# gmarcais/Jellyfish

Hardware: NVIDIA H100
Metric: k-mers counted/sec at k=21 (higher is better)
Workload: dtype u64

## Files before the change

### jellyfish_b200/csrc/jf_engine.cu

```cuda
#include <cuda_runtime.h>
#include <algorithm>
#include <atomic>
#include <cmath>
#include <cstdio>
#include <cstring>
#include <string>
#include <type_traits>
#include <utility>
#include <vector>

#include "../../include/jfgpu.h"
#include "host/jf_matrix.hpp"
#include "jf_kernels.cuh"
#include "jf_extract.cuh"
#include "jf_window.cuh"
#include "jf_dump.cuh"
#include "jf_shard.cuh"
#include "jf_query.cuh"
#include "jf_wide.cuh"
#include "jf_bloom.cuh"
#include "jf_sam.cuh"
#include "jf_newline.cuh"

using namespace jfk;
// ... 399 lines not shown
template<int NTH>
size_t count_smem_bytes(size_t lut_bytes, size_t stage_bytes, size_t bloom_bytes = 0, bool fast = false) {
  const size_t part = fast ? FAST_SMEM : (stage_bytes ? PMAX * 4 + stage_bytes : 0);
  return ((sizeof(ExtractSmemT<NTH>) + 15) & ~(size_t)15) + lut_bytes + part + bloom_bytes;
}

int ensure_scratch(jfgpu_engine* e, uint64_t n_tiles) {
  if(n_tiles <= e->scratch_tiles) return JFGPU_OK;
  uint64_t want = std::max<uint64_t>(n_tiles, 1024);
  CUDA_OK(e, cudaStreamSynchronize(e->cs));
  e->scratch_tiles = 0;
  CUDA_OK(e, make_all(need(e->nlA, want * 8), need(e->nlB, want * 8), need(e->cntA, want * 4), need(e->cntB, want * 4), need(e->tstate, want)));
  e->scratch_tiles = want;
  return JFGPU_OK;
}

uint32_t ring_len_for(uint32_t P) {
  uint32_t p2 = 1; while(p2 < P) p2 <<= 1;
  const uint32_t len = p2 >= RING_P ? RING : RING * (RING_P / p2);
  return std::min<uint32_t>(len, 1024);
}
PartDev part_dev(const jfgpu_engine* e) {
  PartDev d;
  memset(&d, 0, sizeof(d));
  const PartState& ps = e->part;
  d.P = ps.P; d.region_bits = ps.region_bits; d.rec_bytes = ps.rec_bytes; d.cap = ps.cap; d.flush_min = ps.flush_min;
  d.chunk_recs = CHUNK_BYTES / std::max(1u, ps.rec_bytes); d.n_chunks = ps.n_chunks; d.stage_bytes = ps.stage_bytes;
  d.margin = ps.margin;
  d.lazy_win = e->tab.materialized < e->tab.local_size ? e->tab.win_state.as<uint32_t>() : nullptr;
  d.arena_chunks = ps.arena_chunks;
  d.ring_len = ring_len_for(ps.P ? ps.P : 1);
  d.pool = ps.pool.as<uint8_t>(); d.pool_next = ps.pool_next.as<unsigned int>(); d.n_units = d.pool_next + ps.n_arenas; d.dir = ps.dir.as<uint2>();
  d.cta_chunk = ps.cta_chunk.as<uint32_t>(); d.cta_fill = ps.cta_fill.as<uint32_t>();
  d.spill_keys = ps.spill_keys.as<uint64_t>(); d.spill_counts = ps.spill_counts.as<uint64_t>();
  d.spill_n = ps.spill_n.as<unsigned long long>(); d.spill_cap = ps.spill_cap;
  return d;
}

PartDev shard_send_dev(const jfgpu_engine* e, int bank) {
  PartDev d;
  memset(&d, 0, sizeof(d));
  const ShardState& sh = e->sh;
  const uint32_t G = e->p.n_shards;
  d.P = sh.P; d.region_bits = sh.sbits; d.rec_bytes = 4; d.chunk_recs = CHUNK_BYTES / 4;
  d.n_chunks = (uint32_t)(sh.arena_chunks * G); d.arena_chunks = (uint32_t)sh.arena_chunks;
  d.by_owner = 1; d.owner_shift = sh.owner_shift;
  d.ring_len = ring_len_for(sh.P);
  { const double mean = 4096.0 / sh.P; d.margin = std::max<uint32_t>(2 * RING, (uint32_t)(mean + 6.0 * sqrt(mean) + 8.0)); }
  d.pool = sh.send_pool + (size_t)bank * G * sh.arena_chunks * CHUNK_BYTES;
  d.dir = sh.send_dir + (size_t)bank * G * sh.arena_chunks;
  d.pool_next = sh.pool_next[bank].as<unsigned int>(); d.n_units = d.pool_next + G;
  d.cta_chunk = sh.cta_chunk.as<uint32_t>(); d.cta_fill = sh.cta_fill.as<uint32_t>();
  return d;
}

void part_configure(jfgpu_engine* e) {
  PartState& ps = e->part;
  const Table& t = e->tab;
  ps.P = 0;
  if(e->kw == 4) return;
  if(e->p.no_partition || t.bytes() < ((size_t)(e->p.part_min_mb ? e->p.part_min_mb : 256) << 20)) return;
  uint32_t P = 256;
  const size_t region_target = (size_t)(e->p.region_mb ? e->p.region_mb : 64) << 20;
  const size_t owned_bytes = (size_t)t.local_size * (t.slot_bits / 8);
  while(P < (uint32_t)PMAX && (owned_bytes / P) > region_target) P <<= 1;
  if(t.slot_bits == 32 && t.local_lsize > ceil_log2(P)) {
    const uint32_t bits = t.local_lsize - ceil_log2(P) + t.hb, extra = bits > 32 ? bits - 32 : 0;
    if(extra && extra < 8 && (P << extra) <= (uint32_t)RING_P && t.local_lsize - ceil_log2(P << extra) > WIN_LG) P <<= extra;
  }
  for(;; P >>= 1) {
    if(P < 64 || t.local_lsize < 8 || (1u << (t.local_lsize - 8)) < P) return;
    const uint32_t region_bits = t.local_lsize - ceil_log2(P);
    const uint32_t bits = region_bits + t.hb;
    const uint32_t rec = bits <= 32 ? 4 : bits <= 64 ? 8 : bits <= 128 ? 16 : 0;
    if(!rec) return;
    const double mean = 1024.0 * 32 / P;
    const uint32_t margin = (uint32_t)(mean + 6.0 * sqrt(mean) + 8.0);
    if(margin * 2 > CHUNK_BYTES / rec) return;
    ps.P = P; ps.region_bits = region_bits; ps.rec_bytes = rec; ps.cap = 0; ps.flush_min = 0; ps.margin = margin;
    ps.stage_bytes = PMAX * 4;
    return;
  }
}

int part_alloc(jfgpu_engine* e) {
  PartState& ps = e->part;
  if(ps.pool.p) return JFGPU_OK;
  size_t free_b = 0, total_b = 0;
  CUDA_OK(e, cudaMemGetInfo(&free_b, &total_b));
  size_t want = e->p.pool_bytes ? (size_t)e->p.pool_bytes : std::min<size_t>((size_t)(free_b * 0.7), (size_t)64 << 30);
  const size_t floor_b = (size_t)e->n_sm * ps.P * CHUNK_BYTES * 2;
  if(want < floor_b) want = floor_b;
  ps.n_arenas = (uint32_t)e->n_sm;
  ps.arena_chunks = (uint32_t)std::min<size_t>(want / CHUNK_BYTES / ps.n_arenas, 0xFFFFFFF0u / ps.n_arenas);
  ps.n_chunks = ps.arena_chunks * ps.n_arenas;
  ps.spill_cap = (uint64_t)16 << 20;
  if(make_all(need(ps.pool, (size_t)ps.n_chunks * CHUNK_BYTES), need(ps.dir, (size_t)ps.n_chunks * 8), need(ps.order, (size_t)ps.n_chunks * 4),
              need(ps.pool_next, ((size_t)ps.n_arenas + 2) * 4), need(ps.cta_chunk, (size_t)e->n_sm * PMAX * 4),
              need(ps.cta_fill, (size_t)e->n_sm * PMAX * 4), need(ps.spill_keys, ps.spill_cap * 8 * e->kw), need(ps.spill_counts, ps.spill_cap * 8),
              need(ps.spill_n, 8), need(ps.hist, PMAX * 12), need(ps.start, PMAX * 4), need(ps.cursor, PMAX * 4), need(ps.unit_cursor, 8)) != cudaSuccess)
    return fail(e, JFGPU_ERR_NOMEM, "device allocation of the record pool failed");
  CUDA_OK(e, cudaMemsetAsync(ps.pool_next.p, 0, ps.pool_next.bytes, e->cs));
  CUDA_OK(e, cudaMemsetAsync(ps.spill_n.p, 0, 8, e->cs));
  CUDA_OK(e, cudaMemsetAsync(ps.cta_chunk.p, 0xFF, ps.cta_chunk.bytes, e->cs));
  CUDA_OK(e, cudaMemsetAsync(ps.cta_fill.p, 0, ps.cta_fill.bytes, e->cs));
  ps.bound_chunks = ps.P;
  ps.pending = false;
  CUDA_OK(e, cudaStreamSynchronize(e->cs));
  return JFGPU_OK;
}

static unsigned long long* region_recs(PartState& ps) { return reinterpret_cast<unsigned long long*>(ps.hist.as<uint32_t>() + PMAX); }

int regrow(jfgpu_engine* e);
int spill_table(jfgpu_engine* e, uint64_t n_failed);
int read_stats(jfgpu_engine* e);
int bloom_draw(jfgpu_engine* e);
BloomDev bloom_dev(const jfgpu_engine* e);

struct FailWatch {
  jfgpu_engine* e; cudaStream_t st;
  unsigned n = 0;
  bool step(bool last) {
    const int slot = (int)(n++ & 1);
    cudaMemcpyAsync(e->h_watch + slot, e->stats.as<unsigned long long>() + STAT_FAILED, 8, cudaMemcpyDeviceToHost, st);
    cudaEventRecord(e->ev_watch[slot], st);
    return (n > 1 && seen(slot ^ 1)) || (last && seen(slot));
  }
  bool seen(int slot) { cudaEventSynchronize(e->ev_watch[slot]); return e->h_watch[slot] != 0; }
};
static cudaError_t win_event(jfgpu_engine* e, cudaStream_t st) {
  if(e->wev_used == e->wev.size()) e->wev.emplace_back();
  Event& ev = e->wev[e->wev_used];
  if(!ev) { const cudaError_t c = make_all(need(ev, cudaEventDefault)); if(c != cudaSuccess) return c; }
  cudaEventRecord(ev, st);
  e->wev_used++;
  return cudaSuccess;
}
static void resolve_win_events(jfgpu_engine* e, cudaStream_t st) {
  const size_t n_groups = e->wev_used / 4;
  std::vector<uint32_t> flag(n_groups);
  if(n_groups && (cudaMemcpyAsync(flag.data(), e->part.w_flag.p, n_groups * 4, cudaMemcpyDeviceToHost, st) != cudaSuccess ||
                  cudaStreamSynchronize(st) != cudaSuccess)) cudaGetLastError();
  for(size_t j = 0; j < n_groups; ++j)
    for(int q = 0; q < 3; ++q) {
      float ms = 0;
      const int to = q == 0 ? 1 : q == 1 ? (flag[j] ? 0 : 1) : 2;
      if(cudaEventElapsedTime(&ms, e->wev[4 * j + q], e->wev[4 * j + q + 1]) == cudaSuccess) e->win_ms[to] += ms; else cudaGetLastError();
    }
  e->wev_used = 0;
}
static bool window_enabled(jfgpu_engine* e, const PartDev& pd) {
  return (e->p.k2_mode == 0 || e->p.k2_mode == 3 || e->p.k2_mode == 4) && e->op == 0 && e->tab.slot_bits == 32 && pd.rec_bytes == 4 &&
         pd.region_bits > WIN_LG && pd.region_bits - WIN_LG <= 11 && CHUNK_BYTES == (WIN_ST_NTH / 2) * 16;
}
static bool lazy_zero_ok(jfgpu_engine* e) {
  return e->part.P && e->bloom.mode == BLOOM_NONE && window_enabled(e, part_dev(e)) &&
         tri(e->tab.max_reprobe) < ((uint64_t)1 << e->part.region_bits);
}
int part_drain(jfgpu_engine* e, cudaStream_t st) {
  PartState& ps = e->part;
  if(!ps.P || !ps.pool.p || !ps.pending) return JFGPU_OK;
  PartDev pd = part_dev(e);
  const bool win = window_enabled(e, pd);
  const int g = e->n_sm * 4;
  if(!e->ev_d0) CUDA_OK(e, make_all(need(e->ev_d0, cudaEventDefault), need(e->ev_d1, cudaEventDefault)));
  cudaEventRecord(e->ev_d0, st);
  close_chunks_kernel<<<g, 256, 0, st>>>(pd, (uint32_t)e->n_sm); JF_LAUNCHED();
  CUDA_OK(e, cudaMemsetAsync(ps.hist.p, 0, PMAX * 12, st));
  chunk_hist_kernel<<<g, 256, 0, st>>>(pd, ps.hist.as<uint32_t>(), win ? region_recs(ps) : nullptr); JF_LAUNCHED();
  chunk_scan_kernel<<<1, 1024, 0, st>>>(pd.P, ps.hist.as<uint32_t>(), ps.start.as<uint32_t>(), ps.cursor.as<uint32_t>(), pd.n_units); JF_LAUNCHED();
  chunk_scatter_kernel<<<g, 256, 0, st>>>(pd, ps.cursor.as<uint32_t>(), ps.order.as<uint32_t>()); JF_LAUNCHED();
  CUDA_OK(e, cudaMemsetAsync(ps.unit_cursor.p, 0, 8, st));
  const TableDev T0 = table_dev(e, e->tab);
  const bool careful = e->p.allow_regrow != 0 || e->spill_fn != nullptr;
  unsigned int n_units = 0xFFFFFFFFu;
  if(careful || win) {
    CUDA_OK(e, cudaMemcpyAsync(&n_units, pd.n_units, 4, cudaMemcpyDeviceToHost, st));
    CUDA_OK(e, cudaStreamSynchronize(st));
    n_units = std::min(n_units, ps.n_chunks);
  }
  const unsigned group = careful ? (unsigned)std::max<uint64_t>(1, e->fail_group / pd.chunk_recs) : 0xFFFFFFFFu;

  const uint32_t wpr_lg = win ? pd.region_bits - WIN_LG : 0;
  const uint64_t wpr = (uint64_t)1 << wpr_lg;
  const size_t scatter_smem = ((size_t)4 * wpr + (size_t)WIN_ST_UNITS * pd.chunk_recs) * 4;
  std::vector<uint32_t> start(pd.P + 1);
  std::vector<unsigned long long> recs(pd.P);
  auto win_begin = [&]() -> int {
    if(!ps.w_rec.p) {
      ps.w_rec_cap = (uint64_t)64 << 20;
      ps.w_def_cap = WIN_DEF_CAP;
      if(make_all(need(ps.w_rec, ps.w_rec_cap * 4 + 64), need(ps.w_start, (((size_t)WIN_MAX_G << 11) + 1) * 4), need(ps.w_cursor, ((size_t)WIN_MAX_G << 11) * 4),
                  need(ps.w_cnt, ((size_t)WIN_MAX_G << 11) * 4), need(ps.w_def_n, 16), need(ps.w_flag, PMAX * 4),
                  need(ps.w_def_pos[0], ps.w_def_cap * 8), need(ps.w_def_high[0], ps.w_def_cap * 4),
                  need(ps.w_def_pos[1], ps.w_def_cap * 8), need(ps.w_def_high[1], ps.w_def_cap * 4)) != cudaSuccess)
        return fail(e, JFGPU_ERR_NOMEM, "device allocation of the window buffers failed");
      CUDA_OK(e, cudaMemsetAsync(ps.w_def_n.p, 0, 16, st));
    }
    CUDA_OK(e, cudaMemsetAsync(ps.w_flag.p, e->p.k2_mode == 3 ? 1 : 0, PMAX * 4, st));
    CUDA_OK(e, cudaMemcpyAsync(start.data(), ps.start.p, (size_t)pd.P * 4, cudaMemcpyDeviceToHost, st));
    CUDA_OK(e, cudaMemcpyAsync(recs.data(), region_recs(ps), (size_t)pd.P * 8, cudaMemcpyDeviceToHost, st));
    CUDA_OK(e, cudaStreamSynchronize(st));
    start[pd.P] = n_units;
    for(uint32_t r = 0; r < pd.P; ++r) start[r] = std::min(start[r], n_units);
    cudaFuncSetAttribute(win_scatter_kernel<true>, cudaFuncAttributeMaxDynamicSharedMemorySize, (int)scatter_smem);
    cudaFuncSetAttribute(win_scatter_kernel<false>, cudaFuncAttributeMaxDynamicSharedMemorySize, (int)scatter_smem);
    return JFGPU_OK;
  };
  int rc = win ? win_begin() : JFGPU_OK;
  auto bucket_cap = [&](uint64_t m) -> uint64_t {
    const uint64_t c = e->p.k2_mode == 4 ? m : m + (uint64_t)std::ceil(6.0 * std::sqrt((double)m)) + 16;
    return (c + 3) & ~(uint64_t)3;
  };
  bool zero = win && e->tab.materialized == 0;
  int def_wait = -1;
  auto run_deferred = [&](int set) {
    WinDev wd;
    memset(&wd, 0, sizeof(wd));
    wd.def_pos = ps.w_def_pos[set].as<uint64_t>(); wd.def_high = ps.w_def_high[set].as<uint32_t>();
    wd.def_n = ps.w_def_n.as<unsigned long long>() + set; wd.def_cap = ps.w_def_cap;
    if(e->kw == 1) win_deferred_kernel<1><<<e->n_sm * 2, 256, 0, st>>>(T0, wd, e->tab.inv_lut.as<uint64_t>(), e->nbytes);
    else           win_deferred_kernel<2><<<e->n_sm * 2, 256, 0, st>>>(T0, wd, e->tab.inv_lut.as<uint64_t>(), e->nbytes);
    JF_LAUNCHED();
    cudaMemsetAsync(wd.def_n, 0, 8, st);
  };
  auto end_zero = [&]() -> int {
    const int rc2 = table_materialize(e, e->tab, st);
    if(rc2 || !zero) return rc2;
    if(def_wait >= 0) run_deferred(def_wait);
    def_wait = -1; zero = false;
    return JFGPU_OK;
  };
  DevBuf old_inv;
  bool rebuilt = false;
  auto range = [&](unsigned done, unsigned upto) -> int {
    int rc2 = end_zero();
    if(rc2) return rc2;
    cudaMemsetAsync(ps.unit_cursor.p, 0, 8, st);
    const TableDev T = table_dev(e, e->tab);
    if(rebuilt) {
      const size_t smem = (size_t)e->nbytes * 256 * 8 * 2;
      rc2 = dispatch(e, e->kw, e->tab.slot_bits, [&](auto KW, auto SB) -> int {
        auto kern = rehash_chunks_kernel<decltype(KW)::value, decltype(SB)::value>;
        cudaFuncSetAttribute(kern, cudaFuncAttributeMaxDynamicSharedMemorySize, (int)smem);
        kern<<<e->n_sm, 512, smem, st>>>(T, T0, pd, ps.order.as<uint32_t>(), ps.unit_cursor.as<unsigned int>(), done, upto,
                                        old_inv.as<uint64_t>(), e->tab.lut.as<uint64_t>(), e->nbytes);
        return JFGPU_OK;
      });
    } else if(e->op == 0 && e->tab.slot_bits == 32 && pd.rec_bytes == 4 && e->p.k2_mode != 2) {
      if(e->kw == 1) insert_chunks32_kernel<1><<<e->n_sm * 2, 768, 0, st>>>(T, pd, ps.order.as<uint32_t>(), ps.unit_cursor.as<unsigned int>(), done, upto, e->tab.inv_lut.as<uint64_t>(), e->nbytes);
      else           insert_chunks32_kernel<2><<<e->n_sm * 2, 768, 0, st>>>(T, pd, ps.order.as<uint32_t>(), ps.unit_cursor.as<unsigned int>(), done, upto, e->tab.inv_lut.as<uint64_t>(), e->nbytes);
    } else
      rc2 = dispatch(e, e->kw, e->tab.slot_bits, [&](auto KW, auto SB) -> int {
        insert_chunks_kernel<decltype(KW)::value, decltype(SB)::value><<<e->n_sm * 2, 512, 0, st>>>(
            T, pd, ps.order.as<uint32_t>(), ps.unit_cursor.as<unsigned int>(), done, upto, e->tab.inv_lut.as<uint64_t>(), e->nbytes);
        return JFGPU_OK;
      });
    if(!rc2) JF_LAUNCHED();
    return rc2;
  };

  FailWatch watch{e, st};
  unsigned done = 0;
  uint32_t r0 = 0, ng = 0;
  bool ranged = false;
  while(!rc) {
    const bool window = win && !rebuilt;
    if(done >= n_units && (window || ranged)) break;
    unsigned upto = 0;
    if(!window) {
      upto = (unsigned)std::min<uint64_t>((uint64_t)done + group, n_units);
      rc = range(done, upto);
      ranged = true;
    } else {
      WinDev wd;
      memset(&wd, 0, sizeof(wd));
      uint32_t G = 0, stiles = 0;
      uint64_t m = 0, cap = 0;
      while(r0 + G < pd.P && G < WIN_MAX_G) {
        const uint32_t nu = start[r0 + G + 1] - start[r0 + G];
        if(careful && start[r0 + G + 1] - start[r0] > group) break;
        const uint64_t m2 = std::max<uint64_t>(m, (recs[r0 + G] + wpr - 1) / wpr), cap2 = bucket_cap(m2);
        if((G + 1) * wpr * std::max(cap2, m2 + 3) > ps.w_rec_cap) break;
        m = m2; cap = cap2;
        wd.stile_first[G] = stiles; wd.unit_first[G] = start[r0 + G];
        stiles += (nu + WIN_ST_UNITS - 1) / WIN_ST_UNITS;
        ++G;
      }
      if(G == 0) {
        upto = start[r0 + 1]; r0 += 1;
        rc = range(done, upto);
      } else {
        wd.stile_first[G] = stiles; wd.unit_first[G] = start[r0 + G];
        wd.g0 = r0; wd.G = G; wd.wpr_lg = wpr_lg; wd.n_tiles = stiles; wd.cap = (uint32_t)cap;
        wd.overflow = ps.w_flag.as<uint32_t>() + e->wev_used / 4;
        wd.wstart = ps.w_start.as<uint32_t>(); wd.wcursor = ps.w_cursor.as<uint32_t>(); wd.wcnt = ps.w_cnt.as<uint32_t>();
        wd.wrec = ps.w_rec.as<uint32_t>(); wd.wrec_cap = ps.w_rec_cap;
        const int set = zero ? (int)(ng & 1) : 0;
        wd.def_pos = ps.w_def_pos[set].as<uint64_t>(); wd.def_high = ps.w_def_high[set].as<uint32_t>();
        wd.def_n = ps.w_def_n.as<unsigned long long>() + set; wd.def_cap = ps.w_def_cap;
        wd.lazy_win = zero ? e->tab.win_state.as<uint32_t>() : nullptr;
        const uint32_t hb = e->tab.fbits - e->tab.rbits;
        auto settle = [&]() {
          if(!zero) { if(stiles) run_deferred(set); return; }
          e->tab.materialized = (uint64_t)(r0 + G) << pd.region_bits;
          if(def_wait >= 0) run_deferred(def_wait);
          def_wait = stiles ? set : -1;
        };
        ++ng;
        if(stiles) {
          CUDA_OK(e, cudaMemsetAsync(ps.w_cursor.p, 0, ((size_t)G << wpr_lg) * 4, st));
          CUDA_OK(e, win_event(e, st));
          win_scatter_kernel<true><<<stiles, WIN_ST_NTH, scatter_smem, st>>>(pd, wd, ps.order.as<uint32_t>(), hb); JF_LAUNCHED();
          win_scan_kernel<<<1, 1024, 0, st>>>(wd, T0.stats); JF_LAUNCHED();
          CUDA_OK(e, win_event(e, st));
          win_scatter_kernel<false><<<std::min<uint32_t>(stiles, e->n_sm * 2), WIN_ST_NTH, scatter_smem, st>>>(pd, wd, ps.order.as<uint32_t>(), hb);
          JF_LAUNCHED();
          CUDA_OK(e, win_event(e, st));
          if(e->kw == 1) {
            cudaFuncSetAttribute(win_insert2_kernel<1>, cudaFuncAttributeMaxDynamicSharedMemorySize, (int)WIN2_SMEM);
            win_insert2_kernel<1><<<e->n_sm, WIN2_NTH, WIN2_SMEM, st>>>(T0, pd, wd, e->tab.inv_lut.as<uint64_t>(), e->nbytes); JF_LAUNCHED();
          } else {
            cudaFuncSetAttribute(win_insert2_kernel<2>, cudaFuncAttributeMaxDynamicSharedMemorySize, (int)WIN2_SMEM);
            win_insert2_kernel<2><<<e->n_sm, WIN2_NTH, WIN2_SMEM, st>>>(T0, pd, wd, e->tab.inv_lut.as<uint64_t>(), e->nbytes); JF_LAUNCHED();
          }
          if(zero) {
            win_zero_kernel<<<e->n_sm * 4, 256, 0, st>>>(e->tab.slots.as<uint32_t>(), wd.lazy_win, wd.wcnt, (uint64_t)r0 << wpr_lg, G << wpr_lg);
            JF_LAUNCHED();
          }
          settle();
          CUDA_OK(e, win_event(e, st));
        } else {
          if(zero) {
            win_zero_kernel<<<e->n_sm * 4, 256, 0, st>>>(e->tab.slots.as<uint32_t>(), wd.lazy_win, nullptr, (uint64_t)r0 << wpr_lg, G << wpr_lg);
            JF_LAUNCHED();
          }
          settle();
        }
        upto = start[r0 + G]; r0 += G;
      }
    }
    if(rc) break;
    done = upto;
    if(!careful) continue;
    const bool last = done >= n_units;
    if(last) { rc = end_zero(); if(rc) break; }
    if(!watch.step(last)) continue;
    rc = end_zero();
    if(rc) break;
    cudaStreamSynchronize(st);
    watch.n = 0;
    if(!rebuilt) {
      if(old_inv.alloc(e->tab.inv_lut.bytes) != cudaSuccess) { cudaGetLastError(); rc = fail(e, JFGPU_ERR_NOMEM, "device allocation failed"); break; }
      cudaMemcpyAsync(old_inv.p, e->tab.inv_lut.p, e->tab.inv_lut.bytes, cudaMemcpyDeviceToDevice, e->cs);
      cudaStreamSynchronize(e->cs);
      rebuilt = true;
    }
    rc = regrow(e);
  }
  if(!rc) rc = end_zero();
  if(!rc) {
    TableDev T = table_dev(e, e->tab);
    const size_t smem = (size_t)e->nbytes * 256 * 8;
    rc = dispatch(e, e->kw, e->tab.slot_bits, [&](auto KW, auto SB) -> int {
      auto kern = insert_spill_kernel<decltype(KW)::value, decltype(SB)::value>;
      cudaFuncSetAttribute(kern, cudaFuncAttributeMaxDynamicSharedMemorySize, (int)smem);
      kern<<<e->n_sm * 2, 256, smem, st>>>(T, e->tab.lut.as<uint64_t>(), e->nbytes, pd);
      return JFGPU_OK;
    });
    if(!rc) JF_LAUNCHED();
  }
  cudaMemsetAsync(ps.pool_next.p, 0, ps.pool_next.bytes, st);
  cudaMemsetAsync(ps.spill_n.p, 0, 8, st);
  cudaEventRecord(e->ev_d1, st);
  cudaStreamSynchronize(st);
  { float ms = 0; if(cudaEventElapsedTime(&ms, e->ev_d0, e->ev_d1) == cudaSuccess) e->drain_ms += ms; else cudaGetLastError(); }
  resolve_win_events(e, st);
  ps.pending = false;
  if(rebuilt) {
    part_configure(e);
    if(!ps.P) ps = PartState();
  }
  ps.bound_chunks = ps.P;
  if(rc) return rc;
  CUDA_OK(e, cudaGetLastError());
  return JFGPU_OK;
}

uint64_t chunk_usable(const PartState& ps) { return CHUNK_BYTES / ps.rec_bytes - ps.margin; }
uint64_t chunks_for(const PartState& ps, uint64_t per_cta) { return per_cta / chunk_usable(ps) + 2; }

int part_reserve(jfgpu_engine* e, cudaStream_t st, uint64_t need, const char* too_small) {
  PartState& ps = e->part;
  if(ps.bound_chunks + need > ps.arena_chunks) {
    const int rc = part_drain(e, st);
    if(rc || !ps.P) return rc;
  }
  if(ps.bound_chunks + need > ps.arena_chunks) return fail(e, JFGPU_ERR_NOMEM, too_small);
  ps.bound_chunks += need;
  ps.pending = true;
  return JFGPU_OK;
}

size_t part_cap_len(const jfgpu_engine* e, size_t len) {
  const PartState& ps = e->part;
  if(!ps.P || !ps.arena_chunks) return len;
  const uint64_t room = ps.arena_chunks > ps.P + 8 ? ps.arena_chunks - ps.P - 8 : 1;
  const uint64_t tiles_per_cta = std::max<uint64_t>(room * chunk_usable(ps) / (1024 * 32), 1);
  const uint64_t cap = tiles_per_cta * (1024 * 32 - HALO) * (uint64_t)e->n_sm / 2;
  return len > cap ? (size_t)std::max<uint64_t>(cap & ~(uint64_t)15, 16) : len;
}

static uint32_t eff_min_qual(const jfgpu_engine* e) { return e->op == JFGPU_OP_PRIME || e->querying ? 0u : e->p.min_qual; }

enum K1Use : uint32_t {
  K1_COUNT = 0,
  K1_ROUTE = 1,
  K1_SEND = 2,
  K1_QUERY = 4,
};

int run_batch(jfgpu_engine* e, const uint8_t* dev, uint64_t n, uint64_t n_look, cudaStream_t stream, K1Use use, uint64_t n_back = 0,
              int bank = 0, uint64_t* route_keys = nullptr, unsigned long long* route_counts = nullptr, uint64_t route_cap = 0) {
  if(n == 0) return JFGPU_OK;
  PartState& ps = e->part;
  const bool bc_build = e->bloom.mode == BLOOM_COUNT;
  bool part = use == K1_COUNT && ps.P != 0 && !bc_build;
  int rc;
  if(e->bloom.mode != BLOOM_NONE && !e->bloom.drawn && (e->op != JFGPU_OP_PRIME || bc_build)) { rc = bloom_draw(e); if(rc) return rc; }
  if(part) {
    rc = part_alloc(e);
    if(rc) return rc;
    const uint64_t tile_b = 1024 * 32 - HALO;
    const uint64_t tiles = (n + tile_b - 1) / tile_b;
    rc = part_reserve(e, stream, chunks_for(ps, (tiles + e->n_sm - 1) / e->n_sm * tile_b), "record pool smaller than one batch");
    if(rc) return rc;
    part = ps.P != 0;
  }
  if(!part && use == K1_COUNT && !bc_build) {
    rc = table_materialize(e, e->tab, stream);
    if(rc) return rc;
  }
  const bool shard_send = use == K1_SEND;
  const bool query = use == K1_QUERY;
  const uint32_t tile = (part || shard_send ? 1024 : 512) * 32 - HALO;
  const uint64_t n_tiles = (n + tile - 1) / tile;
  rc = ensure_scratch(e, n_tiles);
  if(rc) return rc;
  const int g0 = (int)std::min<uint64_t>(n_tiles, (uint64_t)e->n_sm * 8);
  nl_scan_kernel<<<g0, 256, 0, stream>>>(dev, n, n_tiles, tile, e->nlA.as<long long>(), e->nlB.as<long long>(), e->cntA.as<uint32_t>(), e->cntB.as<uint32_t>());
  JF_LAUNCHED();
  if(e->format == 1)
    tile_state_fastq_kernel<<<1, 1024, 0, stream>>>(n_tiles, e->cntA.as<uint32_t>(), e->cntB.as<uint32_t>(), e->carry[e->carry_cur].as<Carry>(), e->tstate.as<uint8_t>());
  else
    tile_state_kernel<<<1, 1024, 0, stream>>>(dev, n_tiles, tile, e->nlA.as<long long>(), e->nlB.as<long long>(),
                                              e->carry[e->carry_cur].as<Carry>(), e->tstate.as<uint8_t>(), eff_min_qual(e));
  JF_LAUNCHED();
  CountArgs a;
  memset(&a, 0, sizeof(a));
  a.in = dev; a.n = n; a.n_look = n_look; a.n_tiles = n_tiles;
  a.tile_state = e->tstate.as<uint8_t>();
  a.carry_in = e->carry[e->carry_cur].as<Carry>();
  a.carry_out = e->carry[e->carry_cur ^ 1].as<Carry>();
  a.lut = e->tab.hash_fast ? e->tab.lut11.as<uint64_t>() : e->tab.lut.as<uint64_t>();
  a.hash_fast = e->tab.hash_fast ? 1 : 0; a.n_prow = e->tab.n_prow;
  a.lut_bytes = e->tab.hash_fast ? 4 * 2048 * 4 : e->nbytes * 256 * 8;
  for(unsigned i = 0; i < 8; ++i) a.prow[i] = e->tab.prow[i];
  a.min_qual = eff_min_qual(e); a.n_back = n_back;
  a.k = e->k; a.canonical = e->p.canonical; a.nbytes = e->nbytes; a.mode = use; a.format = (uint32_t)e->format;
// ... 1752 lines not shown
```

### jellyfish_b200/csrc/jf_window.cuh

```cuda
#pragma once

namespace jfk {

constexpr uint32_t WIN_MAX_G = 64;
constexpr uint32_t WIN_MAX_WPR = 2048;

struct WinDev {
  uint32_t g0, G, wpr_lg, n_tiles;
  uint32_t cap;
  const uint32_t* lazy_win;
  uint32_t stile_first[WIN_MAX_G + 1];
  uint32_t unit_first[WIN_MAX_G + 1];
  uint32_t* overflow;
  uint32_t* wstart;
  uint32_t* wcursor;
  uint32_t* wcnt;
  uint32_t* wrec; uint64_t wrec_cap;
  uint64_t* def_pos; uint32_t* def_high; unsigned long long* def_n; uint64_t def_cap;
};

__device__ __forceinline__ uint64_t win_slot_base(const WinDev& wd, uint32_t region_bits, uint32_t task) {
  return ((uint64_t)(wd.g0 + (task >> wd.wpr_lg)) << region_bits) + ((uint64_t)(task & ((1u << wd.wpr_lg) - 1)) << WIN_LG);
}

__global__ void __launch_bounds__(1024) win_scan_kernel(WinDev wd, unsigned long long* __restrict__ stats) {
  __shared__ uint32_t part[1024];
  const uint32_t n = wd.G << wd.wpr_lg;
  if(*wd.overflow == 0) {
    for(uint32_t i = threadIdx.x; i < n; i += 1024) { wd.wstart[i] = i * wd.cap; wd.wcnt[i] = wd.wcursor[i]; }
    if(threadIdx.x == 0) wd.wstart[n] = n * wd.cap;
    return;
  }
  const uint32_t per = (n + 1023) / 1024;
  const uint32_t b = threadIdx.x * per, e = min(b + per, n);
  uint32_t s = 0;
  for(uint32_t i = b; i < e; ++i) s += (wd.wcursor[i] + 3u) & ~3u;
  part[threadIdx.x] = s;
  __syncthreads();
  for(uint32_t d = 1; d < 1024; d <<= 1) {
    const uint32_t v = threadIdx.x >= d ? part[threadIdx.x - d] : 0;
    __syncthreads();
    part[threadIdx.x] += v;
    __syncthreads();
  }
  uint32_t run = part[threadIdx.x] - s;
  for(uint32_t i = b; i < e; ++i) {
    const uint32_t c = wd.wcursor[i];
    wd.wstart[i] = run; wd.wcursor[i] = run; wd.wcnt[i] = c;
    run += (c + 3u) & ~3u;
  }
  if(threadIdx.x == 1023) {
    wd.wstart[n] = part[1023];
    if(part[1023] > wd.wrec_cap) atomicAdd(&stats[STAT_POOL_FULL], 1ull);
  }
}

constexpr uint32_t WIN_ST_UNITS = 12;
constexpr uint32_t WIN_ST_NTH = 1024;

template<bool BUCKETS>
__device__ __forceinline__ void win_scatter_tile(const PartDev& pd, const WinDev& wd, const uint32_t* __restrict__ order, uint32_t hb, uint32_t tile) {
  extern __shared__ __align__(16) uint32_t wsm[];
  const uint32_t wpr = 1u << wd.wpr_lg;
  uint32_t* cnt = wsm; uint32_t* lbase = cnt + wpr; uint32_t* lcur = lbase + wpr; uint32_t* gbase = lcur + wpr;
  uint32_t* stage = gbase + wpr;
  __shared__ uint32_t warp_tot[WIN_ST_NTH / 32];
  __shared__ uint32_t s_chunk[WIN_ST_UNITS], s_n[WIN_ST_UNITS];
  __shared__ uint32_t s_skip;
  const uint32_t tid = threadIdx.x;
  for(uint32_t i = tid; i < wpr; i += WIN_ST_NTH) cnt[i] = 0;
  uint32_t r = 0;
  while(r + 1 < wd.G && wd.stile_first[r + 1] <= tile) ++r;
  const uint32_t u0 = wd.unit_first[r] + (tile - wd.stile_first[r]) * WIN_ST_UNITS;
  const uint32_t u1 = min(u0 + WIN_ST_UNITS, wd.unit_first[r + 1]);
  if(tid < WIN_ST_UNITS) {
    uint32_t c = 0, n = 0;
    if(u0 + tid < u1) { c = __ldg(order + u0 + tid); n = __ldg(&pd.dir[c].y); }
    s_chunk[tid] = c; s_n[tid] = n;
  }
  __syncthreads();
  const uint32_t half = tid >> 9, piece = tid & 511u;
  const uint32_t wmask = wpr - 1;
#pragma unroll
  for(uint32_t it = 0; it < WIN_ST_UNITS / 2; ++it) {
    const uint32_t j = 2 * it + half, n = s_n[j];
    if(piece * 4 < n) {
      const uint4 v = __ldg(reinterpret_cast<const uint4*>(pd.pool + (size_t)s_chunk[j] * CHUNK_BYTES) + piece);
      const uint32_t rec[4] = { v.x, v.y, v.z, v.w };
#pragma unroll
      for(uint32_t q = 0; q < 4; ++q) if(piece * 4 + q < n) atomicAdd(&cnt[((rec[q] >> hb) >> WIN_LG) & wmask], 1u);
    }
  }
  __syncthreads();
  const uint32_t per = (wpr + WIN_ST_NTH - 1) / WIN_ST_NTH;
  const uint32_t b = tid * per;
  uint32_t s = 0;
  for(uint32_t i = b; i < min(b + per, wpr); ++i) s += cnt[i];
  uint32_t incl = s;
#pragma unroll
  for(int o = 1; o < 32; o <<= 1) { const uint32_t v = __shfl_up_sync(0xffffffffu, incl, o); if((tid & 31) >= (uint32_t)o) incl += v; }
  if((tid & 31) == 31) warp_tot[tid >> 5] = incl;
  __syncthreads();
  uint32_t woff = 0, total = 0;
  for(uint32_t w = 0; w < WIN_ST_NTH / 32; ++w) { const uint32_t x = warp_tot[w]; if(w < (tid >> 5)) woff += x; total += x; }
  uint32_t run = woff + incl - s;
  for(uint32_t i = b; i < min(b + per, wpr); ++i) {
    const uint32_t c = cnt[i];
    lbase[i] = run; lcur[i] = run;
    uint32_t at = 0;
    if(c) {
      const uint32_t gw = (r << wd.wpr_lg) + i;
      at = atomicAdd(&wd.wcursor[gw], c);
      if(BUCKETS) {
        if(at + c <= wd.cap) at += gw * wd.cap;
        else { at = (uint32_t)wd.wrec_cap; *(volatile uint32_t*)wd.overflow = 1u; }
      }
    }
    gbase[i] = at - run;
    run += c;
  }
  if(BUCKETS && tid == 0) s_skip = *(volatile uint32_t*)wd.overflow;
  __syncthreads();
  if(BUCKETS && s_skip) return;
#pragma unroll
  for(uint32_t it = 0; it < WIN_ST_UNITS / 2; ++it) {
    const uint32_t j = 2 * it + half, n = s_n[j];
    if(piece * 4 < n) {
      const uint4 v = __ldcs(reinterpret_cast<const uint4*>(pd.pool + (size_t)s_chunk[j] * CHUNK_BYTES) + piece);
      const uint32_t rec[4] = { v.x, v.y, v.z, v.w };
#pragma unroll
      for(uint32_t q = 0; q < 4; ++q) if(piece * 4 + q < n) stage[atomicAdd(&lcur[((rec[q] >> hb) >> WIN_LG) & wmask], 1u)] = rec[q];
    }
  }
  __syncthreads();
  for(uint32_t i = tid; i < total; i += WIN_ST_NTH) {
    const uint32_t v = stage[i], w = ((v >> hb) >> WIN_LG) & wmask;
    const uint32_t dst = gbase[w] + i;
    if(dst < wd.wrec_cap) wd.wrec[dst] = v;
  }
}

template<bool BUCKETS>
__global__ void __launch_bounds__(WIN_ST_NTH, 2) win_scatter_kernel(PartDev pd, WinDev wd, const uint32_t* __restrict__ order, uint32_t hb) {
  if constexpr(BUCKETS) {
    win_scatter_tile<true>(pd, wd, order, hb, blockIdx.x);
  } else {
    if(*wd.overflow == 0) return;
    for(uint32_t t = blockIdx.x; t < wd.n_tiles; t += gridDim.x) {
      win_scatter_tile<false>(pd, wd, order, hb, t);
      __syncthreads();
    }
  }
}

constexpr uint32_t WIN2_NTH = 1024;
constexpr uint32_t WIN2_CONS = WIN2_NTH - 32;
constexpr uint32_t WIN2_RB  = 10240;
constexpr uint32_t WIN2_BLK = 256;
constexpr uint32_t WIN2_NONE = 0xFFFFFFFFu;
constexpr size_t   WIN2_SMEM = (size_t)2 * WIN_SLOTS * 4 + (size_t)2 * WIN2_RB * 4;

struct Win2Info { uint32_t task, b, n, pad; };

template<int KW>
__global__ void __launch_bounds__(WIN2_NTH, 1) win_insert2_kernel(TableDev T, PartDev pd, WinDev wd, const uint64_t* __restrict__ inv_lut_g, uint32_t nbytes) {
  extern __shared__ __align__(128) uint8_t w2smem[];
  __shared__ __align__(8) uint64_t full[2];
  __shared__ __align__(8) uint64_t empty[2];
  __shared__ Win2Info info[2];
  __shared__ uint32_t cursor[2];
  uint32_t* const winb0 = reinterpret_cast<uint32_t*>(w2smem);
  uint32_t* const recb0 = winb0 + 2 * WIN_SLOTS;
  uint32_t* tab = (uint32_t*)T.slots;
  const uint32_t n_tasks = wd.G << wd.wpr_lg;
  const uint32_t tid = threadIdx.x, lane = tid & 31u;

  auto slot_base_of = [&](uint32_t task) -> uint64_t { return win_slot_base(wd, pd.region_bits, task); };
  if(tid == 0) {
    mbar_init(&full[0], 1); mbar_init(&full[1], 1);
    mbar_init(&empty[0], WIN2_CONS / 32); mbar_init(&empty[1], WIN2_CONS / 32);
    fence_proxy_async();
  }
  __syncthreads();

  if(tid < 32) {
    const bool lead = lane == 0;
    uint32_t next_from = blockIdx.x;
    uint32_t ephase[2] = { 0, 0 };
    uint32_t cur_task[2] = { WIN2_NONE, WIN2_NONE }, cur_n[2] = { 0, 0 }, cur_b[2] = { 0, 0 };
    auto load_batch = [&](uint32_t s, uint32_t off, bool with_window) {
      const uint32_t nb = min(WIN2_RB, cur_n[s] - off);
      const uint32_t rbytes = ((nb + 3u) & ~3u) * 4u;
      cursor[s] = 0;
      mbar_expect_tx(&full[s], rbytes + (with_window ? WIN_SLOTS * 4u : 0u));
      if(with_window) tma_load_1d(winb0 + s * WIN_SLOTS, tab + slot_base_of(cur_task[s]), WIN_SLOTS * 4u, &full[s]);
      tma_load_1d(recb0 + s * WIN2_RB, wd.wrec + cur_b[s] + off, rbytes, &full[s]);
    };
    auto next_window = [&](uint32_t s) {
      uint32_t t = next_from, c = 0;
      while(t < n_tasks && (c = wd.wcnt[t]) == 0) t += gridDim.x;
      if(t >= n_tasks) {
        next_from = t; cur_task[s] = WIN2_NONE;
        if(lead) { info[s].task = WIN2_NONE; mbar_arrive(&full[s]); }
        return;
      }
      next_from = t + gridDim.x;
      cur_task[s] = t; cur_n[s] = c; cur_b[s] = wd.wstart[t];
      const bool fill = wd.lazy_win && wd.lazy_win[slot_base_of(t) >> WIN_LG] != WIN_IN_MEMORY;
      if(fill) {
        uint4* const w = reinterpret_cast<uint4*>(winb0 + s * WIN_SLOTS);
        for(uint32_t i = lane; i < WIN_SLOTS / 4; i += 32) w[i] = make_uint4(0, 0, 0, 0);
        fence_proxy_async();
        __syncwarp();
      }
      if(lead) {
        info[s].task = t; info[s].b = cur_b[s]; info[s].n = c;
        load_batch(s, 0, !fill);
      }
    };
    next_window(0); next_window(1);
    for(uint32_t s = 0; cur_task[s] != WIN2_NONE; s ^= 1u) {
      for(uint32_t off = WIN2_RB; off < cur_n[s]; off += WIN2_RB) {
        mbar_wait(&empty[s], ephase[s]); ephase[s] ^= 1u;
        if(lead) load_batch(s, off, false);
      }
      mbar_wait(&empty[s], ephase[s]); ephase[s] ^= 1u;
      if(lead) {
        tma_store_1d(tab + slot_base_of(cur_task[s]), winb0 + s * WIN_SLOTS, WIN_SLOTS * 4u);
        tma_commit_group();
        tma_wait_group_read0();
      }
      __syncwarp();
      next_window(s);
    }
    if(lead) tma_wait_group0();
    return;
  }

  const uint32_t fb = T.fbits, rb = T.rbits, hb = fb - rb;
  const uint32_t fmask = (1u << fb) - 1u, one = 1u << fb, cb = 32 - fb;
  const uint32_t hmask = hb ? ((1u << hb) - 1u) : 0u;
  const uint32_t lt_mask = (1u << lane) - 1u;
  uint32_t n_ins = 0, n_new = 0, n_rep = 0;
  uint32_t fphase[2] = { 0, 0 };
  for(uint32_t s = 0; ; s ^= 1u) {
    mbar_wait(&full[s], fphase[s]); fphase[s] ^= 1u;
    const Win2Info inf = info[s];
    if(inf.task == WIN2_NONE) break;
    uint32_t* const win = winb0 + s * WIN_SLOTS;
    const uint32_t* const recs = recb0 + s * WIN2_RB;
    const uint64_t slot_base = slot_base_of(inf.task);
    for(uint32_t off = 0; off < inf.n; off += WIN2_RB) {
      const uint32_t nb = min(WIN2_RB, inf.n - off);
      if(off) { mbar_wait(&full[s], fphase[s]); fphase[s] ^= 1u; }
      bool have = false, want = true;
      uint32_t rec = 0, local = 0, kf = 0, at = 0, p = 0;
      uint32_t blk_next = 0, blk_end = 0;
      bool more = true;
      for(;;) {
        const uint32_t need = __ballot_sync(0xffffffffu, want);
        if(need && more) {
          if(blk_next >= blk_end) {
            uint32_t base = 0;
            if(lane == 0) base = atomicAdd(&cursor[s], WIN2_BLK);
            blk_next = __shfl_sync(0xffffffffu, base, 0);
            blk_end = min(blk_next + WIN2_BLK, nb);
            more = blk_next < nb;
          }
          if(want && more) {
            const uint32_t i = blk_next + __popc(need & lt_mask);
            if(i < blk_end) {
              rec = recs[i];
              local = (rec >> hb) & (WIN_SLOTS - 1); kf = ((rec & hmask) << rb) | 1u;
              at = local; p = 0;
              have = true; want = false;
            }
          }
          blk_next = min(blk_next + (uint32_t)__popc(need), blk_end);
        }
        if(!__any_sync(0xffffffffu, have)) { if(!more) break; else continue; }
        if(have) {
          if(at < WIN_SLOTS) {
            const uint32_t o = atomicCAS(&win[at], 0u, kf | one);
            if(o == 0u) { ++n_new; ++n_ins; n_rep += p; want = true; }
            else if((o & fmask) == kf) {
              const uint32_t o2 = atomicAdd(&win[at], one);
              if((((o2 >> fb) + 1) >> cb) != 0) k2_carry(T.ovf_keys, T.ovf_vals, T.ovf_mask, T.stats, slot_base + at);
              ++n_ins; n_rep += p; want = true;
            } else if(p < T.max_reprobe) { ++p; at += p; ++kf; }
            else {
              k2_fail<KW>(T.shard_index, T.local_lsize, T.lsize, T.stats, T.fail_keys, T.fail_counts, T.fail_cap, slot_base + local, rec & hmask, inv_lut_g, nbytes);
              want = true;
            }
          } else {
            const unsigned long long d = atomicAdd(wd.def_n, 1ull);
            if(d < wd.def_cap) { wd.def_pos[d] = slot_base + local; wd.def_high[d] = rec & hmask; }
            else atomicAdd(&T.stats[STAT_POOL_FULL], 1ull);
            want = true;
          }
          have = !want;
        }
      }
      fence_proxy_async();
      __syncwarp();
      if(lane == 0) mbar_arrive(&empty[s]);
// ... 33 lines not shown
```

Before: 43.58 billion.

## Rewrite window scatter as persistent TMA double-buffered kernel with single chunk read

The window scatter kernel becomes persistent, one CTA per SM, looping over tiles. Chunks are prefetched into shared memory with TMA bulk loads on mbarriers, double-buffered so the next tile loads while the current one is processed. Records are read from global memory once instead of twice, and packed per-record atomic ranks replace the second atomic pass through a separate staging area. The cost is lower occupancy (launch bounds drop from 2 CTAs to 1), more complex mbarrier synchronisation, and removal of the chunk-size guard in window_enabled.

Result: faster. 44.93 billion (median of 6 runs) (+3.1%).

```diff
diff --git a/jellyfish_b200/csrc/jf_engine.cu b/jellyfish_b200/csrc/jf_engine.cu
--- a/jellyfish_b200/csrc/jf_engine.cu
+++ b/jellyfish_b200/csrc/jf_engine.cu
@@ -575,7 +575,7 @@
 }
 static bool window_enabled(jfgpu_engine* e, const PartDev& pd) {
   return (e->p.k2_mode == 0 || e->p.k2_mode == 3 || e->p.k2_mode == 4) && e->op == 0 && e->tab.slot_bits == 32 && pd.rec_bytes == 4 &&
-         pd.region_bits > WIN_LG && pd.region_bits - WIN_LG <= 11 && CHUNK_BYTES == (WIN_ST_NTH / 2) * 16;
+         pd.region_bits > WIN_LG && pd.region_bits - WIN_LG <= 11;
 }
 static bool lazy_zero_ok(jfgpu_engine* e) {
   return e->part.P && e->bloom.mode == BLOOM_NONE && window_enabled(e, part_dev(e)) &&
@@ -607,7 +607,7 @@
 
   const uint32_t wpr_lg = win ? pd.region_bits - WIN_LG : 0;
   const uint64_t wpr = (uint64_t)1 << wpr_lg;
-  const size_t scatter_smem = ((size_t)4 * wpr + (size_t)WIN_ST_UNITS * pd.chunk_recs) * 4;
+  const size_t scatter_smem = win_scatter_smem(WIN_ST_UNITS, WIN_ST_NBUF, (uint32_t)wpr);
   std::vector<uint32_t> start(pd.P + 1);
   std::vector<unsigned long long> recs(pd.P);
   auto win_begin = [&]() -> int {
@@ -735,10 +735,10 @@
         if(stiles) {
           CUDA_OK(e, cudaMemsetAsync(ps.w_cursor.p, 0, ((size_t)G << wpr_lg) * 4, st));
           CUDA_OK(e, win_event(e, st));
-          win_scatter_kernel<true><<<stiles, WIN_ST_NTH, scatter_smem, st>>>(pd, wd, ps.order.as<uint32_t>(), hb); JF_LAUNCHED();
+          win_scatter_kernel<true><<<std::min<uint32_t>(stiles, e->n_sm), WIN_ST_NTH, scatter_smem, st>>>(pd, wd, ps.order.as<uint32_t>(), hb); JF_LAUNCHED();
           win_scan_kernel<<<1, 1024, 0, st>>>(wd, T0.stats); JF_LAUNCHED();
           CUDA_OK(e, win_event(e, st));
-          win_scatter_kernel<false><<<std::min<uint32_t>(stiles, e->n_sm * 2), WIN_ST_NTH, scatter_smem, st>>>(pd, wd, ps.order.as<uint32_t>(), hb);
+          win_scatter_kernel<false><<<std::min<uint32_t>(stiles, e->n_sm), WIN_ST_NTH, scatter_smem, st>>>(pd, wd, ps.order.as<uint32_t>(), hb);
           JF_LAUNCHED();
           CUDA_OK(e, win_event(e, st));
           if(e->kw == 1) {
diff --git a/jellyfish_b200/csrc/jf_window.cuh b/jellyfish_b200/csrc/jf_window.cuh
--- a/jellyfish_b200/csrc/jf_window.cuh
+++ b/jellyfish_b200/csrc/jf_window.cuh
@@ -56,101 +56,161 @@
 }
 
 constexpr uint32_t WIN_ST_UNITS = 12;
+constexpr uint32_t WIN_ST_NBUF = 2;
 constexpr uint32_t WIN_ST_NTH = 1024;
 
+__host__ __device__ constexpr size_t win_scatter_smem(uint32_t units, uint32_t nbuf, uint32_t wpr) {
+  return (size_t)nbuf * units * CHUNK_BYTES + (size_t)3 * wpr * 4;
+}
+static_assert(win_scatter_smem(WIN_ST_UNITS, WIN_ST_NBUF, WIN_MAX_WPR) + 1024 <= 227 * 1024, "one CTA per SM");
+
+template<bool BUCKETS, uint32_t UNITS, uint32_t NBUF, uint32_t NTH>
+__device__ __forceinline__ void win_scatter_tiles(const PartDev& pd, const WinDev& wd, const uint32_t* __restrict__ order, uint32_t hb) {
+  constexpr uint32_t CR = CHUNK_BYTES / 4;
+  constexpr uint32_t V = UNITS * (CHUNK_BYTES / 16) / NTH;
+  constexpr uint32_t PER_MAX = NTH >= WIN_MAX_WPR ? 1 : NTH * 2 >= WIN_MAX_WPR ? 2 : 4;
+  static_assert(UNITS * (CHUNK_BYTES / 16) % NTH == 0 && NTH % 32 == 0 && NTH * PER_MAX >= WIN_MAX_WPR && NBUF >= 2 && UNITS <= 32, "tile shape");
+  static_assert(UNITS * CR <= 65536, "ranks are packed two to a word");
+  extern __shared__ __align__(128) uint32_t wsm[];
+  __shared__ __align__(8) uint64_t full[NBUF];
+  __shared__ uint32_t s_n[NBUF][UNITS];
+  __shared__ uint32_t warp_tot[NTH / 32];
+  __shared__ uint32_t s_skip;
+  if(!BUCKETS && *wd.overflow == 0) return;
+  const uint32_t wpr = 1u << wd.wpr_lg, wmask = wpr - 1;
+  uint32_t per_lg = 0;
+  while((NTH << per_lg) < wpr) ++per_lg;
+  const uint32_t per = 1u << per_lg;
+  uint32_t* const cnt = wsm + NBUF * UNITS * CR;
+  uint32_t* const lbase = cnt + wpr;
+  uint32_t* const gbase = lbase + wpr;
+  const uint32_t tid = threadIdx.x, lane = tid & 31u, warp = tid >> 5;
+  const uint32_t n_mine = blockIdx.x < wd.n_tiles ? (wd.n_tiles - 1 - blockIdx.x) / gridDim.x + 1 : 0;
+  auto region_of = [&](uint32_t tile) { uint32_t r = 0; while(r + 1 < wd.G && wd.stile_first[r + 1] <= tile) ++r; return r; };
+  auto chunk_of = [&](uint32_t k) -> uint32_t {
+    if(k >= n_mine || lane >= UNITS) return NO_CHUNK;
+    const uint32_t tile = blockIdx.x + k * gridDim.x, r = region_of(tile);
+    const uint32_t u = wd.unit_first[r] + (tile - wd.stile_first[r]) * UNITS + lane;
+    return u < wd.unit_first[r + 1] ? __ldg(order + u) : NO_CHUNK;
+  };
+  auto recs_of = [&](uint32_t c) -> uint32_t { return c != NO_CHUNK ? min(__ldg(&pd.dir[c].y), CR) : 0u; };
+  auto issue = [&](uint32_t k, uint32_t c, uint32_t n) {
+    const uint32_t b = k % NBUF, bytes = ((n + 3u) & ~3u) * 4u;
+    uint32_t sum = bytes;
+#pragma unroll
+    for(int o = 16; o; o >>= 1) sum += __shfl_xor_sync(0xffffffffu, sum, o);
+    if(lane < UNITS) s_n[b][lane] = n;
+    __syncwarp();
+    if(lane == 0) { fence_proxy_async(); mbar_expect_tx(&full[b], sum); }
+    __syncwarp();
+    if(bytes) tma_load_1d(wsm + (b * UNITS + lane) * CR, pd.pool + (size_t)c * CHUNK_BYTES, bytes, &full[b]);
+  };
+
+  if(tid == 0) {
+    for(uint32_t b = 0; b < NBUF; ++b) mbar_init(&full[b], 1);
+    fence_proxy_async();
+    s_skip = 0;
+  }
+  for(uint32_t i = tid; i < wpr; i += NTH) cnt[i] = 0;
+  __syncthreads();
+  uint32_t pc = NO_CHUNK, pn = 0;
+  if(warp == 0) {
+    for(uint32_t k = 0; k + 1 < NBUF && k < n_mine; ++k) { const uint32_t c = chunk_of(k); issue(k, c, recs_of(c)); }
+    pc = chunk_of(NBUF - 1); pn = recs_of(pc);
+  }
+  bool skip = false;
+
+  for(uint32_t k = 0; k < n_mine; ++k) {
+    const uint32_t b = k % NBUF;
+    uint32_t* const buf = wsm + b * UNITS * CR;
+    mbar_wait(&full[b], (k / NBUF) & 1u);
+    uint32_t rec[4 * V], rank[2 * V];
+#pragma unroll
+    for(uint32_t v = 0; v < V; ++v) {
+      const uint32_t x = tid + v * NTH, j = x / (CR / 4), q0 = (x % (CR / 4)) * 4, n = s_n[b][j];
+      const uint4 r4 = reinterpret_cast<const uint4*>(buf)[x];
+      rec[4 * v] = r4.x; rec[4 * v + 1] = r4.y; rec[4 * v + 2] = r4.z; rec[4 * v + 3] = r4.w;
+      rank[2 * v] = rank[2 * v + 1] = 0;
+#pragma unroll
+      for(uint32_t q = 0; q < 4; ++q)
+        if(q0 + q < n) rank[2 * v + q / 2] |= atomicAdd(&cnt[((rec[4 * v + q] >> hb) >> WIN_LG) & wmask], 1u) << (16 * (q & 1));
+    }
+    __syncthreads();
+    if(warp == 0 && k + NBUF - 1 < n_mine) { issue(k + NBUF - 1, pc, pn); pc = chunk_of(k + NBUF); }
+    const uint32_t i0 = tid << per_lg;
+    uint32_t c[PER_MAX], s = 0;
+#pragma unroll
+    for(uint32_t p = 0; p < PER_MAX; ++p) { c[p] = p < per && i0 < wpr ? cnt[i0 + p] : 0u; s += c[p]; }
+    uint32_t incl = s;
+#pragma unroll
+    for(int o = 1; o < 32; o <<= 1) { const uint32_t v = __shfl_up_sync(0xffffffffu, incl, o); if(lane >= (uint32_t)o) incl += v; }
+    if(lane == 31) warp_tot[warp] = incl;
+    if(i0 < wpr) {
+      uint32_t x = incl - s;
+#pragma unroll
+      for(uint32_t p = 0; p < PER_MAX; ++p) if(p < per) { lbase[i0 + p] = x; x += c[p]; cnt[i0 + p] = 0; }
+    }
+    __syncthreads();
+    const uint32_t wt = lane < NTH / 32 ? warp_tot[lane] : 0u;
+    uint32_t winc = wt;
+#pragma unroll
+    for(int o = 1; o < 32; o <<= 1) { const uint32_t v = __shfl_up_sync(0xffffffffu, winc, o); if(lane >= (uint32_t)o) winc += v; }
+    const uint32_t wexcl = winc - wt, total = __shfl_sync(0xffffffffu, winc, 31);
+    const uint32_t run0 = __shfl_sync(0xffffffffu, wexcl, warp) + incl - s;
+    const uint32_t r = region_of(blockIdx.x + k * gridDim.x);
+    uint32_t at[PER_MAX];
+    auto claim = [&] {
+#pragma unroll
+      for(uint32_t p = 0; p < PER_MAX; ++p) at[p] = c[p] ? atomicAdd(&wd.wcursor[(r << wd.wpr_lg) + i0 + p], c[p]) : 0u;
+    };
+    if(BUCKETS) claim();
+    uint32_t flag = 0;
+    if(BUCKETS && tid == 0) flag = *(volatile uint32_t*)wd.overflow;
+    if(!skip) {
+#pragma unroll
+      for(uint32_t v = 0; v < V; ++v) {
+        const uint32_t x = tid + v * NTH, j = x / (CR / 4), q0 = (x % (CR / 4)) * 4, n = s_n[b][j];
+#pragma unroll
+        for(uint32_t q = 0; q < 4; ++q) {
+          const uint32_t w = ((rec[4 * v + q] >> hb) >> WIN_LG) & wmask;
+          const uint32_t off = __shfl_sync(0xffffffffu, wexcl, (w >> per_lg) >> 5);
+          if(q0 + q < n) buf[lbase[w] + off + ((rank[2 * v + q / 2] >> (16 * (q & 1))) & 0xFFFFu)] = rec[4 * v + q];
+        }
+      }
+    }
+    if(!BUCKETS) claim();
+    if(i0 < wpr) {
+      uint32_t run = run0;
+#pragma unroll
+      for(uint32_t p = 0; p < PER_MAX; ++p) if(p < per) {
+        uint32_t a = at[p];
+        if(BUCKETS && c[p]) {
+          const uint32_t gw = (r << wd.wpr_lg) + i0 + p;
+          if(a + c[p] <= wd.cap) a += gw * wd.cap;
+          else { a = (uint32_t)wd.wrec_cap; *(volatile uint32_t*)wd.overflow = 1u; flag = 1; }
+        }
+        gbase[i0 + p] = a - run;
+        run += c[p];
+      }
+    }
+    if(BUCKETS && flag) s_skip = 1;
+    fence_proxy_async();
+    __syncthreads();
+    if(BUCKETS) skip = s_skip != 0;
+    if(!skip) {
+      for(uint32_t i = tid; i < total; i += NTH) {
+        const uint32_t v = buf[i], w = ((v >> hb) >> WIN_LG) & wmask;
+        const uint32_t dst = gbase[w] + i;
+        if(dst < wd.wrec_cap) wd.wrec[dst] = v;
+      }
+    }
+    if(warp == 0) pn = recs_of(pc);
+  }
+}
+
 template<bool BUCKETS>
-__device__ __forceinline__ void win_scatter_tile(const PartDev& pd, const WinDev& wd, const uint32_t* __restrict__ order, uint32_t hb, uint32_t tile) {
-  extern __shared__ __align__(16) uint32_t wsm[];
-  const uint32_t wpr = 1u << wd.wpr_lg;
-  uint32_t* cnt = wsm; uint32_t* lbase = cnt + wpr; uint32_t* lcur = lbase + wpr; uint32_t* gbase = lcur + wpr;
-  uint32_t* stage = gbase + wpr;
-  __shared__ uint32_t warp_tot[WIN_ST_NTH / 32];
-  __shared__ uint32_t s_chunk[WIN_ST_UNITS], s_n[WIN_ST_UNITS];
-  __shared__ uint32_t s_skip;
-  const uint32_t tid = threadIdx.x;
-  for(uint32_t i = tid; i < wpr; i += WIN_ST_NTH) cnt[i] = 0;
-  uint32_t r = 0;
-  while(r + 1 < wd.G && wd.stile_first[r + 1] <= tile) ++r;
-  const uint32_t u0 = wd.unit_first[r] + (tile - wd.stile_first[r]) * WIN_ST_UNITS;
-  const uint32_t u1 = min(u0 + WIN_ST_UNITS, wd.unit_first[r + 1]);
-  if(tid < WIN_ST_UNITS) {
-    uint32_t c = 0, n = 0;
-    if(u0 + tid < u1) { c = __ldg(order + u0 + tid); n = __ldg(&pd.dir[c].y); }
-    s_chunk[tid] = c; s_n[tid] = n;
-  }
-  __syncthreads();
-  const uint32_t half = tid >> 9, piece = tid & 511u;
-  const uint32_t wmask = wpr - 1;
-#pragma unroll
-  for(uint32_t it = 0; it < WIN_ST_UNITS / 2; ++it) {
-    const uint32_t j = 2 * it + half, n = s_n[j];
-    if(piece * 4 < n) {
-      const uint4 v = __ldg(reinterpret_cast<const uint4*>(pd.pool + (size_t)s_chunk[j] * CHUNK_BYTES) + piece);
-      const uint32_t rec[4] = { v.x, v.y, v.z, v.w };
-#pragma unroll
-      for(uint32_t q = 0; q < 4; ++q) if(piece * 4 + q < n) atomicAdd(&cnt[((rec[q] >> hb) >> WIN_LG) & wmask], 1u);
-    }
-  }
-  __syncthreads();
-  const uint32_t per = (wpr + WIN_ST_NTH - 1) / WIN_ST_NTH;
-  const uint32_t b = tid * per;
-  uint32_t s = 0;
-  for(uint32_t i = b; i < min(b + per, wpr); ++i) s += cnt[i];
-  uint32_t incl = s;
-#pragma unroll
-  for(int o = 1; o < 32; o <<= 1) { const uint32_t v = __shfl_up_sync(0xffffffffu, incl, o); if((tid & 31) >= (uint32_t)o) incl += v; }
-  if((tid & 31) == 31) warp_tot[tid >> 5] = incl;
-  __syncthreads();
-  uint32_t woff = 0, total = 0;
-  for(uint32_t w = 0; w < WIN_ST_NTH / 32; ++w) { const uint32_t x = warp_tot[w]; if(w < (tid >> 5)) woff += x; total += x; }
-  uint32_t run = woff + incl - s;
-  for(uint32_t i = b; i < min(b + per, wpr); ++i) {
-    const uint32_t c = cnt[i];
-    lbase[i] = run; lcur[i] = run;
-    uint32_t at = 0;
-    if(c) {
-      const uint32_t gw = (r << wd.wpr_lg) + i;
-      at = atomicAdd(&wd.wcursor[gw], c);
-      if(BUCKETS) {
-        if(at + c <= wd.cap) at += gw * wd.cap;
-        else { at = (uint32_t)wd.wrec_cap; *(volatile uint32_t*)wd.overflow = 1u; }
-      }
-    }
-    gbase[i] = at - run;
-    run += c;
-  }
-  if(BUCKETS && tid == 0) s_skip = *(volatile uint32_t*)wd.overflow;
-  __syncthreads();
-  if(BUCKETS && s_skip) return;
-#pragma unroll
-  for(uint32_t it = 0; it < WIN_ST_UNITS / 2; ++it) {
-    const uint32_t j = 2 * it + half, n = s_n[j];
-    if(piece * 4 < n) {
-      const uint4 v = __ldcs(reinterpret_cast<const uint4*>(pd.pool + (size_t)s_chunk[j] * CHUNK_BYTES) + piece);
-      const uint32_t rec[4] = { v.x, v.y, v.z, v.w };
-#pragma unroll
-      for(uint32_t q = 0; q < 4; ++q) if(piece * 4 + q < n) stage[atomicAdd(&lcur[((rec[q] >> hb) >> WIN_LG) & wmask], 1u)] = rec[q];
-    }
-  }
-  __syncthreads();
-  for(uint32_t i = tid; i < total; i += WIN_ST_NTH) {
-    const uint32_t v = stage[i], w = ((v >> hb) >> WIN_LG) & wmask;
-    const uint32_t dst = gbase[w] + i;
-    if(dst < wd.wrec_cap) wd.wrec[dst] = v;
-  }
-}
-
-template<bool BUCKETS>
-__global__ void __launch_bounds__(WIN_ST_NTH, 2) win_scatter_kernel(PartDev pd, WinDev wd, const uint32_t* __restrict__ order, uint32_t hb) {
-  if constexpr(BUCKETS) {
-    win_scatter_tile<true>(pd, wd, order, hb, blockIdx.x);
-  } else {
-    if(*wd.overflow == 0) return;
-    for(uint32_t t = blockIdx.x; t < wd.n_tiles; t += gridDim.x) {
-      win_scatter_tile<false>(pd, wd, order, hb, t);
-      __syncthreads();
-    }
-  }
+__global__ void __launch_bounds__(WIN_ST_NTH, 1) win_scatter_kernel(PartDev pd, WinDev wd, const uint32_t* __restrict__ order, uint32_t hb) {
+  win_scatter_tiles<BUCKETS, WIN_ST_UNITS, WIN_ST_NBUF, WIN_ST_NTH>(pd, wd, order, hb);
 }
 
 constexpr uint32_t WIN2_NTH = 1024;
```
